# zhangyp15/MonoFlex

Hardware: AMD Instinct MI355X
Metric: images/sec at 1280x384, DLA-34+DCNv2 forward+decode (higher is better)
Workload: dtype bf16; 1 GPU; DLA-34+DCNv2+9 heads+edge fusion forward + NMS/top-K/3D decode, batch 8 per GPU, 1280x384, bf16 (BASELINE.json configs[1]); batch_per_gpu=8, launch=hipGraph, parallelism=replicas x1 (no collective on the inference path), sub_batch_streams=1, detections_last_step=400, h2d_excluded=True, d2h_excluded=True

## Files before the change

### include/monoflex_hip.h

```cpp
#ifndef MONOFLEX_HIP_H
#define MONOFLEX_HIP_H

#include <stddef.h>
#include <stdint.h>

#ifdef __cplusplus
extern "C" {
#endif

#define MFX_ABI_VERSION 3

enum { MFX_F32 = 0, MFX_BF16 = 1, MFX_F16 = 2 ,
       MFX_F16X2 = 3  };
enum { MFX_ACT_NONE = 0, MFX_ACT_RELU = 1, MFX_ACT_LEAKY = 2 , MFX_ACT_DCN_OFFMASK = 3  };
enum { MFX_OK = 0, MFX_ERR_ARG = -1, MFX_ERR_UNSUPPORTED = -2, MFX_ERR_LAUNCH = -3, MFX_ERR_WORKSPACE = -4 };

int mfx_abi_version(void);
const char* mfx_last_error(void);
int mfx_set_option(const char* name, int value);
int mfx_reset_options(void);
int mfx_commit_options(void);
long mfx_get_counter(const char* name);

int mfx_f16x2_range_check(int reset);
// ... 111 lines not shown
int mfx_nchw_to_nhwc(const float* x, void* y, int B, int C, int H, int W, int ldy, int dtype, void* stream);
int mfx_nhwc_to_nchw(const void* x, float* y, int B, int C, int H, int W, int ldx, int dtype, void* stream);
int mfx_pack_image_nhwc4(const float* x, void* y, int B, int H, int W, int pad_h, int pad_w_left, int pad_w_right,
                         int dtype, void* stream);

typedef struct {
    const void* x;
    const void* w1;
    const float* scale1; const float* shift1;
    const void* w2;
    const float* bias2;
    float* out;
    float* planar;
    int32_t B, H, W, nbranch, K_pad, ld_out, dtype, planar_c;
    int32_t ch_off[16]; int32_t c_out[16];
    float w2_scale[16];
    const void* w1_32; const void* w2_32;
} mfx_heads_desc;
int mfx_heads_fused(const mfx_heads_desc* d, void* stream);

int mfx_edge_scatter_add(float* out, int ld_out, int ch_off, int C, const float* v, int ldv,
                         const int32_t* edge_xy, const int32_t* edge_len, int B, int L, int H, int W,
                         float* planar , void* stream);

size_t mfx_decode_topk_workspace_bytes(int ncls, int B, int K);
int mfx_decode_topk(const float* hmap, long b_stride, long c_stride, long p_stride, int ncls, int B, int H, int W, int K,
                    float* scores, int32_t* index, void* workspace, size_t workspace_bytes, void* stream);

int mfx_decode_boxes(const float* hmap, int ld, int reg_off, const float* scores, const int32_t* index,
                     int ncls, int B, int H, int W, int K, const float* calib, const int32_t* pad,
                     const int32_t* img_size, float threshold, float* det, float* topk, int32_t* valid,
                     void* stream);
enum { MFX_DEPTH_SOFT = 0, MFX_DEPTH_HARD = 1, MFX_DEPTH_MEAN = 2, MFX_DEPTH_DIRECT = 3, MFX_DEPTH_KEYPOINTS_AVG = 4,
       MFX_DEPTH_KEYPOINTS_CENTER = 5, MFX_DEPTH_KEYPOINTS_02 = 6, MFX_DEPTH_KEYPOINTS_13 = 7 };
int mfx_decode_boxes_mode(const float* hmap, int ld, int reg_off, const float* scores, const int32_t* index,
                          int ncls, int B, int H, int W, int K, const float* calib, const int32_t* pad,
                          const int32_t* img_size, float threshold, int depth_mode, float* det, float* topk, int32_t* valid,
                          void* stream);
typedef struct mfx_decode_cfg {
    float dim_mean[9], dim_std[9];
    float depth_ref[2], depth_range[2];
    float down_ratio, eps;
    int depth_decode;
    int dim_exp, dim_use_std;
    int uncertainty_as_conf;
    int output_depth;
// ... 235 lines not shown
```

### monoflex_amd/build.py

```python
import hashlib
import os
import subprocess
import sys
from concurrent.futures import ThreadPoolExecutor

HERE = os.path.dirname(os.path.abspath(__file__))
CSRC = os.path.join(HERE, "csrc")
OBJ = os.path.join(CSRC, "build")
LIB = os.path.join(CSRC, "libmonoflex_hip.so")
SOURCES = ["capi.hip", "options.hip", "conv_kernels.hip", "conv_halo.hip", "conv_cw.hip", "conv_cws.hip", "misc_kernels.hip", "stem.hip", "f1_fused.hip", "heads.hip", "decode.hip", "dcn_wave.hip", "dcn_patch.hip", "dcn_lds.hip", "dcn_ps.hip", "gemm_as.hip", "dcn_ext.hip", "dcn_bwd.hip", "dcn_bwd_tile.hip", "psroi_pool.hip", "train_kernels.hip", "adamw.hip", "wgrad_tr.hip", "loss_kernels.hip", "box3d_iou.hip", "head_sparse.hip", "gram_heads.hip", "kitti_encode.hip", "kitti_eval.hip"]
FLAGS = ["--offload-arch=gfx950", "-O3", "-std=c++17", "-fPIC", "-Wall", "-Wno-unused-function"]
if os.environ.get("MFX_PROBES") == "1":
    FLAGS.append("-DMFX_PROBES")
EXTRA_FLAGS = {"kitti_encode.hip": ["-ffp-contract=off"], "kitti_eval.hip": ["-ffp-contract=off"],
               "dcn_bwd_tile.hip": ["-fno-slp-vectorize"]}


def _hipcc():
    return "/opt/rocm/bin/hipcc" if os.path.exists("/opt/rocm/bin/hipcc") else "hipcc"


def _headers_digest():
    h = hashlib.sha1()
    for root in (CSRC, os.path.join(os.path.dirname(HERE), "include")):
        for fn in sorted(os.listdir(root)):
            if fn.endswith(".h"):
                with open(os.path.join(root, fn), "rb") as f:
                    h.update(fn.encode() + f.read())
    return h.hexdigest()


def _source_stamp(src, headers):
    h = hashlib.sha1()
# ... 47 lines not shown
```

### monoflex_amd/csrc/options.h

```cpp
#pragma once

#define MFX_NOLO (-2147483647 - 1)
#define MFX_NOHI 2147483647

#define MFX_OPTION_LIST(X) \
     \
    X(conv_tile, 0, MFX_NOLO, MFX_NOHI, "implicit-GEMM tile of mfx_conv2d_nhwc: 0 = automatic, else a tile id (conv_kernels.hip: 1 = 256x16, 2 = 256x32, 3 = 128x64, " \
        "4 = 64x64, 5 = 128x128, 6 = 64x128, 7 = 256x64, 8 = 256x128 / 8 waves, 9 = 128x128 / 8 waves), taken where it fits Cout_pad") \
    X(dcn_tile, 0, MFX_NOLO, MFX_NOHI, "the same for the fused gather DCN kernel") \
    X(cat_tile, 0, MFX_NOLO, MFX_NOHI, "the same for mfx_cat_conv1x1_nhwc") \
    X(kc, 0, MFX_NOLO, MFX_NOHI, "16-byte chunks per LDS row of the implicit-GEMM main loop: 0 = automatic (8 where K_pad allows), 4 = force 4") \
    X(ksplit, 0, MFX_NOLO, MFX_NOHI, "split-K of mfx_conv2d_nhwc: 0 = automatic (never: measured neutral-to-slower on DLA level4/5), 1 = never split, " \
        "n = force n splits where legal") \
    X(dcn_ksplit, 0, MFX_NOLO, MFX_NOHI, "the same for the fused DCN kernel") \
    X(halo, 1, MFX_NOLO, MFX_NOHI, "LDS-staged halo kernels for 3x3 convs: 0 = generic kernel only, 1 = automatic, >= 2 = force variant (value - 1)") \
    X(halo_cg, 0, MFX_NOLO, MFX_NOHI, "max channels per patch pass of the halo kernel (0 = default)") \
    X(halo_s2, 1, MFX_NOLO, MFX_NOHI, "0 = stride-2 3x3 convs stay on the generic implicit-GEMM kernel") \
    X(halo_pair, 1, MFX_NOLO, MFX_NOHI, "split precision walks K in step pairs where mfx_conv_desc.w_frag_pair is given (0 = two mma_chunk per pair)") \
    X(halo_cw, 1, MFX_NOLO, MFX_NOHI, "0 = conv3x3_wave_kernel only, 1 = the compile-time-geometry kernel (conv_cw.hip) where an instantiation exists") \
    X(cw_rows6, 1, MFX_NOLO, MFX_NOHI, "0 = 8-row tiles everywhere in conv_cw.hip (1: 6-row tiles where Ho % 6 == 0, Ho % 8 != 0, Ho <= 48)") \
    X(halo_cws, 1, MFX_NOLO, MFX_NOHI, "0 = conv3x3_wave_kernel<f32s_t> only, 1 = the compile-time-geometry split-precision kernel (conv_cws.hip) where an instantiation exists") \
     \
    X(dcn_wave, 1, MFX_NOLO, MFX_NOHI, "0 = first-generation kernel only, 1 = automatic, 2.. = force variant") \
    X(dcn_patch, 1, MFX_NOLO, MFX_NOHI, "LDS-patch DCN kernel: 0 = off, 1 = automatic, 2 = force (FM 4), 3 = force FM 2, 4 = force FM 1, 5-7 = wide margin FM 4/2/1, " \
        "8 = padded layout") \
    X(dcn_patch_fn8, 1, MFX_NOLO, MFX_NOHI, "1 = one workgroup of the LDS-patch kernel covers 128 output channels where Cout_pad % 128 == 0") \
    X(dcn_fuse_off, 1, MFX_NOLO, MFX_NOHI, "1 = the LDS-patch kernel computes the offset/mask conv itself where the caller supplies its weights") \
    X(dcn_lds, 1, MFX_NOLO, MFX_NOHI, "0 = off, 1 = automatic (64 -> 64 on large 16-bit maps), 2 = wherever the kernel applies") \
    X(dcn_lds_rows, 16, MFX_NOLO, MFX_NOHI, "tile rows, 16 | 8 (three workgroups per CU; measured slower: 2.570 vs 2.551 ms per step, profiles/r06_dcn_lds.md)") \
     \
    X(heads_persist, 1, MFX_NOLO, MFX_NOHI, "1 = one workgroup per resident slot (n > 1: n workgroups), each a contiguous range of (tile, branch) units; " \
        "0 = one workgroup per tile.  B=8 bf16: 516 -> 503 us (tools/probes/heads_probe.py), bit-identical output") \
    X(heads_mfma32, 0, MFX_NOLO, MFX_NOHI, "1 = the v_mfma_f32_32x32x16 form of the kernel where the caller supplies its packs (mfx_heads_desc.w1_32 / w2_32)") \
    X(heads_planes, 0, MFX_NOLO, MFX_NOHI, "1 = four k-group planes (no LDS bank conflicts: 48 % -> 11 % of the LDS cycles, LDS-active cycles -42 %), " \
        "0 = one 144-byte record per pixel.  Same kernel time (555 vs 555 us, A/B in one run): not LDS-bound") \
    X(topk_strips, 8, MFX_NOLO, MFX_NOHI, "row strips per (class, image) map when a workspace is supplied; 1 = single-workgroup kernel") \
    X(topk_merge_z, 16, MFX_NOLO, MFX_NOHI, "workgroups per (class, image) map in the merge; values outside 1..64 are an error") \
    X(topk_merge_threads, 512, MFX_NOLO, MFX_NOHI, "their size; must be a multiple of 64 in 64..512 (the merge ranks by whole wavefronts; 512 = its __launch_bounds__)") \
     \
    X(wgrad_mfma, 1, MFX_NOLO, MFX_NOHI, "0 = VALU kernel for bf16 too, 1 = 64x64 MFMA tiles, 3 = 128x128 where they fit") \
    X(wgrad_blocks, 600, MFX_NOLO, MFX_NOHI, "target workgroup count of the MFMA weight-gradient kernel (measured, B=8 step: 64 -> 146 ms, 150 -> 90, 300 -> 78, " \
        "600 -> 73, 2048 -> 75, 8192 -> 81: the tile atomics of every slab cost more than the extra workgroups hide)") \
    X(wgrad_ws, 1, MFX_NOLO, MFX_NOHI, "0 = always accumulate the tiles with atomics") \
    X(wgrad_ws_blocks, 1200, MFX_NOLO, MFX_NOHI, "target workgroup count when partial tiles go to the workspace (step: 1200 -> 58.0 ms, 2400 -> 58.3, 4800 -> 58.6; " \
        "atomics: 59.6)") \
    X(wgrad_min_m, 128, MFX_NOLO, MFX_NOHI, "fewest pixels of a slab of the MFMA weight-gradient kernel.  r06: 1024 left the 1x1 / Root layers of the 24x80 and 12x40 " \
        "maps with 8-16 slabs (120-240 workgroups of 32 iterations each: 31 us per layer for 4 GFLOP); same-box step 17.50 (1024) / 17.31 (512) / 17.27 (256) / " \
        "17.23-17.31 (128) / 17.26 (64) ms") \
    X(wgrad_tr, 1, MFX_NOLO, MFX_NOHI, "0 = first-generation kernel everywhere (2: the transposed-read kernel also where Cout % 128 != 0)") \
    X(wgrad_tr_blocks, 512, 1, MFX_NOHI, "target workgroup count (tiles x pixel slabs)") \
    X(wgrad_patch, 1, MFX_NOLO, MFX_NOHI, "0 = off (the 3x3 / s1 / p1 weight-gradient form with the input patch in LDS)") \
    X(wgrad_patch_blocks, 256, 1, MFX_NOHI, "target workgroup count") \
    X(wgrad_patch_waves, 12, MFX_NOLO, MFX_NOHI, "6 (64 x 96 block per wave) or 12 (64 x 48)") \
    X(stem_wgrad_blocks, 512, 1, MFX_NOHI, "target workgroup count of the stem's weight-gradient kernel (mfx_stem_wgrad_16)") \
     \
    X(bn_apply_blocks, 1024, MFX_NOLO, MFX_NOHI, "workgroup cap of the two-launch forms' streaming kernels") \
    X(bn_blocks, 768, MFX_NOLO, MFX_NOHI, "target workgroup count of the column reductions (BN statistics / backward sums / bias sums)") \
    X(bn_onepass, 3, MFX_NOLO, MFX_NOHI, "bit 0 = backward, bit 1 = forward in one launch where the map fits (0 = the two-launch forms everywhere)") \
// ... 14 lines not shown
     \
    X(deterministic, 0, MFX_NOLO, MFX_NOHI, "any non-zero value = 1: every floating-point reduction of the training path runs in a fixed order (single-writer partial " \
        "sums, one pixel slab per weight-gradient tile, 64-bit fixed-point accumulation of the DCN input gradient) so that two runs -- eager or replayed from a " \
        "hipGraph -- produce bit-identical results.  Slower; the default (0) keeps the atomics")

#define MFX_PROBE_OPTION_LIST(X) \
    X(dcn_bt_dbg, 0, MFX_NOLO, MFX_NOHI, "experiment switches of dcn_bwd_tile_kernel (0 in production)") \
    X(heads_dbg, 0, MFX_NOLO, MFX_NOHI, "timing probes of the bf16 heads kernel (see DBG in heads.hip)")

#define MFX_COUNTER_LIST(X) \
     \
    X(dcn_lds, "launches of the fourth-generation DCN kernel (dcn_lds.hip) on 16-bit maps") \
    X(dcn_lds_of, "those of dcn_lds that computed the offset/mask conv themselves") \
    X(dcn_lds_split, "launches of dcn_lds.hip in split precision (not counted in dcn_lds)") \
    X(dcn_patch, "launches of the third-generation, LDS-patch DCN kernel (dcn_patch.hip)") \
    X(dcn_wave, "launches of the second-generation DCN kernel (dcn_wave.hip)") \
    X(dcn_gather, "launches of the first-generation fused gather DCN kernel (conv_kernels.hip)") \
    X(conv_cw, "launches of the compile-time-geometry 3x3 kernel (conv_cw.hip)") \
    X(conv_cws, "launches of its split-precision form (conv_cws.hip)") \
    X(conv_halo, "launches of the LDS-staged halo kernel (conv_halo.hip)") \
    X(conv_igemm, "launches of the generic implicit-GEMM kernel (conv_kernels.hip)") \
    X(conv_splitk, "those that ran split-K") \
    X(conv_bn_stats, "convolutions whose epilogue accumulated the BatchNorm statistics") \
     \
    X(wgrad_patch, "weight gradients by the LDS-patch kernel (wgrad_tr.hip)") \
    X(wgrad_tr, "weight gradients by the transposed-read kernel (wgrad_tr.hip)") \
    X(wgrad_mfma, "weight gradients by the first-generation MFMA kernel (train_kernels.hip)") \
    X(wgrad_valu, "weight gradients by the VALU kernel") \
    X(wgrad_reduce, "launches of the pass that sums their partial tiles (wgrad_reduce_kernel)") \
    X(stem_wgrad, "launches of the stem's weight-gradient kernel") \
    X(bn_fwd_onepass, "train-mode BatchNorm forwards in one launch") \
    X(bn_bwd_onepass, "BatchNorm backwards in one launch") \
    X(bn_fwd_two, "BatchNorm forwards in the two-launch form") \
    X(bn_bwd_two, "BatchNorm backwards in the two-launch form") \
    X(dcn_bt_fly, "DCN backward calls that took the gcol-free form") \
    X(dcn_bt_fused, "launches of dcn_bwd_sample_wgrad_kernel") \
    X(dcn_bt_tile, "launches of dcn_bwd_tile_kernel") \
    X(dcn_bt_sample, "launches of dcn_bwd_sample_kernel") \
    X(dcn_bt_far, "launches of dcn_bwd_far_kernel + dcn_bwd_far_fly_kernel") \
    X(gram, "phase calls of mfx_gram_heads on 16-bit maps") \
    X(adamw_multi, "calls of mfx_adamw_multi")

#define MFX_DECLARE_OPTION(name, def, lo, hi, doc) extern int g_opt_##name;
#define MFX_DECLARE_COUNTER(name, doc) extern long g_cnt_##name;
MFX_OPTION_LIST(MFX_DECLARE_OPTION)
MFX_PROBE_OPTION_LIST(MFX_DECLARE_OPTION)
// ... 4 lines not shown
```

### monoflex_amd/lib.py

```python
import ctypes
import os

HERE = os.path.dirname(os.path.abspath(__file__))
LIB_PATH = os.environ.get("MFX_LIB_PATH") or os.path.join(HERE, "csrc", "libmonoflex_hip.so")

MFX_F32, MFX_BF16, MFX_F16, MFX_F16X2 = 0, 1, 2, 3
ACT_NONE, ACT_RELU, ACT_LEAKY, ACT_DCN_OFFMASK = 0, 1, 2, 3
MAX_SEG = 9

c_int, c_void_p, c_float, c_size_t = ctypes.c_int32, ctypes.c_void_p, ctypes.c_float, ctypes.c_size_t


class ConvDesc(ctypes.Structure):
    _fields_ = [("x", c_void_p), ("w", c_void_p), ("w_frag", c_void_p), ("scale", c_void_p), ("shift", c_void_p), ("res", c_void_p),
                ("y", c_void_p), ("rowmap", c_void_p),
                ("B", c_int), ("H", c_int), ("W", c_int), ("x_pixstride", c_int), ("Ck", c_int),
                ("kh", c_int), ("kw", c_int), ("stride", c_int), ("pad_h", c_int), ("pad_w", c_int), ("dil_w", c_int),
                ("Ho", c_int), ("Wo", c_int), ("M", c_int), ("Cout", c_int), ("Cout_pad", c_int), ("K_pad", c_int),
                ("ldy", c_int), ("ldres", c_int), ("act", c_int), ("dtype", c_int), ("out_dtype", c_int),
                ("workspace", c_void_p), ("workspace_bytes", ctypes.c_int64),
                ("stats", c_void_p), ("stats_ncopy", c_int), ("stats_done", ctypes.POINTER(c_int)), ("w_frag_pair", c_void_p)]


class CatDesc(ctypes.Structure):
# ... 2 lines not shown
                ("w", c_void_p), ("scale", c_void_p), ("shift", c_void_p), ("res", c_void_p), ("y", c_void_p),
                ("M", c_int), ("Cout", c_int), ("Cout_pad", c_int), ("K_pad", c_int), ("ldy", c_int),
                ("ldres", c_int), ("act", c_int), ("dtype", c_int)]


class DcnDesc(ctypes.Structure):
    _fields_ = [("x", c_void_p), ("offmask", c_void_p), ("w", c_void_p), ("scale", c_void_p), ("shift", c_void_p),
                ("y", c_void_p), ("w_frag", c_void_p),
                ("B", c_int), ("H", c_int), ("W", c_int), ("C", c_int),
                ("kh", c_int), ("kw", c_int), ("stride", c_int), ("pad", c_int), ("dil", c_int),
                ("Ho", c_int), ("Wo", c_int), ("Cout", c_int), ("Cout_pad", c_int), ("K_pad", c_int),
                ("ldy", c_int), ("act", c_int), ("dtype", c_int), ("w_frag_f16", c_void_p),
                ("workspace", c_void_p), ("workspace_bytes", ctypes.c_int64),
                ("off_w_frag_f16", c_void_p), ("off_shift", c_void_p), ("offmask_out", c_void_p),
                ("nonsquare", c_int), ("stride_w", c_int), ("pad_w", c_int), ("dil_w", c_int), ("w_pair_f16", c_void_p)]


class HeadsDesc(ctypes.Structure):
    _fields_ = [("x", c_void_p), ("w1", c_void_p), ("scale1", c_void_p), ("shift1", c_void_p), ("w2", c_void_p),
                ("bias2", c_void_p), ("out", c_void_p), ("planar", c_void_p),
                ("B", c_int), ("H", c_int), ("W", c_int), ("nbranch", c_int), ("K_pad", c_int), ("ld_out", c_int),
                ("dtype", c_int), ("planar_c", c_int), ("ch_off", c_int * 16), ("c_out", c_int * 16), ("w2_scale", ctypes.c_float * 16),
                ("w1_32", c_void_p), ("w2_32", c_void_p)]


class KittiDesc(ctypes.Structure):
    _fields_ = [(n, c_void_p) for n in (
        "records", "n_obj", "P", "img_wh", "flip", "hm", "cls_ids", "target_centers", "keypoints", "keypoints_depth_mask",
        "dimensions", "locations", "reg_mask", "reg_weight", "offset_3D", "bboxes", "gt_bboxes", "rotys", "trunc_mask", "alphas",
        "orientations", "occlusions", "truncations", "pad_size", "edge_indices", "edge_len", "P_out", "heat_radius", "status")] + \
        [(n, c_int) for n in ("B", "max_objs", "in_w", "in_h", "down", "num_classes")] + \
        [(n, ctypes.c_double) for n in ("filter_trunc", "filter_size", "edge_ratio")]


class KittiEvalDesc(ctypes.Structure):
    _fields_ = [(n, c_void_p) for n in ("gt", "dt", "gt_off", "dt_off", "pair_off", "classes", "min_overlaps", "overlaps", "tp_scores",
                                        "num_valid_gt", "thresholds", "num_thresholds", "pr")] + \
        [(n, c_int) for n in ("B", "n_gt", "n_dt", "num_classes", "num_k", "compute_aos")] + [("n_pairs", ctypes.c_int64)]


class AdamWDesc(ctypes.Structure):
    _fields_ = [("p", c_void_p), ("g", c_void_p), ("m", c_void_p), ("v", c_void_p), ("step", c_void_p), ("numel", ctypes.c_longlong),
                ("group", c_int), ("pad_", c_int)]


class AdamWGroup(ctypes.Structure):
# ... 53 lines not shown
    "mfx_reset_options": (_I, []),
    "mfx_commit_options": (_I, []),
    "mfx_get_counter": (ctypes.c_long, [ctypes.c_char_p]),
    "mfx_f16x2_range_check": (ctypes.c_int, [ctypes.c_int]),
    "mfx_dcn_v2_workspace_bytes": (_S, [_I] * 14),
    "mfx_dcn_v2_workspace_bytes_g": (_S, [_I] * 15),
    "mfx_dcn_v2_forward": (_I, [_P] * 6 + [_I] * 14 + [_P, _S, _P]),
    "mfx_dcn_v2_backward": (_I, [_P] * 11 + [_I] * 14 + [_P, _S, _P]),
    "mfx_dcn_v2_psroi_pooling_forward": (_I, [_P] * 5 + [_I] * 8 + [_F] + [_I] * 5 + [_F, _P]),
    "mfx_dcn_v2_psroi_pooling_backward": (_I, [_P] * 7 + [_I] * 8 + [_F] + [_I] * 5 + [_F, _P]),
    "mfx_conv2d_nhwc": (_I, [ctypes.POINTER(ConvDesc), _P]),
    "mfx_cat_conv1x1_nhwc": (_I, [ctypes.POINTER(CatDesc), _P]),
    "mfx_dcn_nhwc": (_I, [ctypes.POINTER(DcnDesc), _P]),
    "mfx_dcn_sample_nhwc": (_I, [_P, _P, _P, _P, _P, _I, _I, _I, _I, _I, _I, _I, _P]),
    "mfx_project_nhwc": (_I, [_P, _P, _P, _I, _I, _I, _I, _I, _I, _P]),
    "mfx_maxpool2x2_nhwc": (_I, [_P, _P, _I, _I, _I, _I, _I, _P]),
    "mfx_upsample_add_nhwc": (_I, [_P, _P, _P, _P, _I, _I, _I, _I, _I, _I, _P]),
    "mfx_nchw_to_nhwc": (_I, [_P, _P, _I, _I, _I, _I, _I, _I, _P]),
    "mfx_nhwc_to_nchw": (_I, [_P, _P, _I, _I, _I, _I, _I, _I, _P]),
    "mfx_pack_image_nhwc4": (_I, [_P, _P, _I, _I, _I, _I, _I, _I, _I, _P]),
    "mfx_heads_fused": (_I, [ctypes.POINTER(HeadsDesc), _P]),
    "mfx_dcn_fuses_offset_conv": (_I, [ctypes.POINTER(DcnDesc)]),
    "mfx_edge_scatter_add": (_I, [_P, _I, _I, _I, _P, _I, _P, _P, _I, _I, _I, _I, _P, _P]),
    "mfx_decode_topk_workspace_bytes": (_S, [_I, _I, _I]),
    "mfx_decode_topk": (_I, [_P, ctypes.c_long, ctypes.c_long, ctypes.c_long, _I, _I, _I, _I, _I, _P, _P, _P, _S, _P]),
    "mfx_conv_wgrad_nhwc": (_I, [_P, _P, _P] + [_I] * 15 + [_P]),
    "mfx_conv_wgrad_nhwc_dil": (_I, [_P, _P, _P] + [_I] * 16 + [_P]),
    "mfx_conv_wgrad_oihw": (_I, [_P, _P, _P] + [_I] * 17 + [_P, _S, _P]),
    "mfx_pack_conv_weight": (_I, [_P, _I, _I, _I, _I, _I, _P, _P, _I, _I, _I, _I, _P]),
    "mfx_adamw_chunk_elems": (_I, []),
    "mfx_adamw_multi": (_I, [_P, _P, _I, ctypes.c_longlong, _P, _P, _P]),
    "mfx_colsum": (_I, [_P, _P, ctypes.c_long, _I, _I, _I, _P]),
    "mfx_colsum_add": (_I, [_P, _P, ctypes.c_long, _I, _I, _I, _P]),
    "mfx_bn_stats": (_I, [_P, _P, _P, ctypes.c_long, _I, _I, _P]),
    "mfx_bn_finalize": (_I, [_P, _P, _P, _P, _P, _P, _F, _F, ctypes.c_long, _P, _P, _P, _P, _I, _P]),
    "mfx_bn_act_fwd": (_I, [_P, _P, _P, _P, _P, ctypes.c_long, _I, _I, _I, _P]),
    "mfx_bn_act_bwd": (_I, [_P] * 10 + [ctypes.c_long, _I, _I, _I, _P]),
    "mfx_stem_wgrad_bf16": (_I, [_P, _P, _P, _I, _I, _I, _I, _I, _P, _S, _P]),
    "mfx_stem_wgrad_16": (_I, [_P, _P, _P, _I, _I, _I, _I, _I, _I, _P, _S, _P]),
    "mfx_pack_chunk_elems": (_I, []),
    "mfx_pack_conv_weights_batched": (_I, [_P, _P, _I, ctypes.c_longlong, _I, _P]),
    "mfx_head_sparse_fwd": (_I, [ctypes.POINTER(HeadSparseDesc), _P]),
    "mfx_head_sparse_bwd": (_I, [ctypes.POINTER(HeadSparseDesc), _P]),
    "mfx_gram_heads": (_I, [ctypes.POINTER(GramDesc), _I, _P]),
    "mfx_bn_train_stats": (_I, [_P] * 6 + [_F, _F, ctypes.c_long, _I, _I, _P, _P, _P, _I, _P]),
    "mfx_bn_scratch_bytes": (_S, []),
# ... 130 lines not shown
```

### monoflex_amd/model/head/detector_predictor.py

```python
import numpy as np
import torch
from torch import nn

from ... import autograd as AG
from ... import lib as L
from ... import ops

HM_LD = 64
REG_OFF = 8


GRAM_HEADS = [__import__("os").environ.get("MFX_GRAM_HEADS", "1") != "0"]
GRAM_OFFSET = [__import__("os").environ.get("MFX_GRAM_OFFSET", "1") != "0"]


class InPlaceABN(nn.Module):

    def __init__(self, num_features, eps=1e-5, momentum=0.1, affine=True, activation="leaky_relu", activation_param=0.01):
        super().__init__()
        if not affine:
            raise NotImplementedError("InPlaceABN holder: affine=True only")
        self.num_features, self.eps, self.momentum, self.affine, self.track_running_stats = num_features, eps, momentum, True, True
        self.weight = nn.Parameter(torch.ones(num_features))
        self.bias = nn.Parameter(torch.zeros(num_features))
# ... 78 lines not shown
        lasts = [[self.class_head[2]]] + [list(h) for h in self.reg_heads]
        c_out = [sum(h.weight.shape[0] for h in heads) for heads in lasts]
        ch_off = [0] + [REG_OFF + sum(c_out[1:i]) for i in range(1, len(lasts))]
        assert ch_off[-1] + c_out[-1] <= HM_LD
        p = ops.pack_heads([t[0].weight for t in trunks], [self._abn_fold(t[1]) for t in trunks],
                           [torch.cat([h.weight for h in heads]) for heads in lasts], [torch.cat([h.bias for h in heads]) for heads in lasts],
                           self.num_classes, ch_off, HM_LD, dtype)
        if self.enable_edge_fusion:
            oi = self.offset_index[0]
            w_e = torch.cat((self.class_head[0].weight, self.reg_features[oi][0].weight), 0)
            s0, b0 = self._abn_fold(self.class_head[1])
            s1, b1 = self._abn_fold(self.reg_features[oi][1])
            p.edge_trunk = ops.pack_conv(w_e, dtype, torch.cat((s0, s1)), torch.cat((b0, b1)), stride=1, pad=1, act=L.ACT_LEAKY)
            p.edge_branches = []
            for seq, cout, choff in ((self.trunc_heatmap_conv, self.num_classes, 0),
                                     (self.trunc_offset_conv, 2, REG_OFF + sum(sum(c) for c in self.regression_channel_cfg[:oi])
                                      + sum(self.regression_channel_cfg[oi][:self.offset_index[1]]))):
                c1, bn, c3 = seq[0], seq[1], seq[3]
                scale, shift = ops.fold_bn(bn, c1.bias)
                pk1 = ops.pack_conv(c1.weight.detach().unsqueeze(2), dtype, scale, shift, stride=1, pad=0,
                                    act=L.ACT_RELU if self.edge_fusion_relu else L.ACT_NONE)
                pk2 = ops.pack_conv(c3.weight.detach().unsqueeze(2), dtype, None, c3.bias, stride=1, pad=0, act=L.ACT_NONE, cout=4)
                p.edge_branches.append((pk1, pk2, cout, choff))
        self._packs[key] = p
        return p

    def forward_nhwc(self, features, edge_indices=None, edge_lens=None, edge_rowmap=None):
        if self.training:
            raise RuntimeError("forward_nhwc is the fused eval path; training goes through forward_train")
        p = self._pack(ops.compute_tag(self, features.dtype))
        hm, planar = ops.heads_fused(features, p, planar_classes=self.num_classes)
        self.last_cls_planar = planar
        if self.enable_edge_fusion:
            if edge_indices is None:
                raise ValueError("edge fusion is enabled: targets must carry edge_indices / edge_len")
            B, H, W, _ = features.shape
            Lmax = edge_indices.shape[1]
            rowmap = edge_rowmap if edge_rowmap is not None else make_edge_rowmap(edge_indices, H, W)
            trunk = ops.conv2d(features, p.edge_trunk, rowmap=rowmap)
            trunk = trunk.view(B, 1, Lmax + 2, 2 * self.head_conv)
            for bi, (pk1, pk2, cout, choff) in enumerate(p.edge_branches):
                f1 = ops.conv2d(trunk, pk1, x_ch_off=bi * self.head_conv)
                o = ops.conv2d(f1, pk2, out_dtype=torch.float32)
                ops.edge_scatter_add(hm, choff, cout, o, edge_indices, edge_lens, planar=planar if choff == 0 else None)
        return hm

    def forward_train(self, features, edge_indices=None, edge_lens=None, object_rows=None, plan=None):
        B, H, W, _ = features.shape
        trunks = [self.class_head] + list(self.reg_features)
        lasts = [[self.class_head[2]]] + [list(h) for h in self.reg_heads]
        oi = self.offset_index[0]
        sparse = object_rows is not None
        feats, outs, sp = [], [], []
        gram = sparse and GRAM_HEADS[0]
        fuse_nodes = self.enable_edge_fusion and self.fused_edge_nodes
        gram_off = gram and GRAM_OFFSET[0] and (fuse_nodes or not self.enable_edge_fusion)
        is_sparse = lambda bi: sparse and bi != 0 and (bi - 1 != oi or gram_off)
        dense_ids = [bi for bi in range(len(trunks)) if not (gram and is_sparse(bi))]
        ys = dict(zip(dense_ids, AG.fanout_conv(features, [trunks[bi][0].weight for bi in dense_ids], 1)))
        edge_rows = {}
# ... 180 lines not shown
```

### monoflex_amd/ops.py

```python
import ctypes
import os
from typing import Optional

import torch

from . import lib as L
from .packing import (F16X2, STEM_PAD_H, STEM_PAD_WL, STEM_PAD_WR, PackedCat, PackedConv, PackedHeads, _elems, _pad_rows_cols, _pow2,
                      _round_up, add_f16_fragments, cast_operand, compute_tag, cout_pad, dcn_pair_fragments, dcn_ps_pack, fold_bn, fragment_major,
                      pack_cat, pack_conv, pack_heads, pack_stem, pack_upsample, pair_steps, split_chunks, split_halves, split_weight_scale, storage_dtype)


def _stream():
    return ctypes.c_void_p(torch.cuda.current_stream().cuda_stream)


def _first_cuda_device(args):
    for a in args:
        if torch.is_tensor(a):
            if a.is_cuda:
                return a.device
        elif isinstance(a, (list, tuple)):
            d = _first_cuda_device(a)
            if d is not None:
                return d
    return None


def on_tensor_device(fn):
    import functools

    @functools.wraps(fn)
    def run(*args, **kwargs):
# ... 271 lines not shown
@on_tensor_device
def heads_fused(x, p: PackedHeads, planar_classes=0):
    _need_cuda(x)
    B, H, W, C = x.shape
    assert C == 64
    out = torch.empty((B, H, W, p.ld_out), dtype=torch.float32, device=x.device)
    planar = torch.empty((B, planar_classes, H * W), dtype=torch.float32, device=x.device) if planar_classes else None
    d = L.HeadsDesc()
    d.planar, d.planar_c = (planar.data_ptr() if planar is not None else None), planar_classes
    d.x, d.w1, d.scale1, d.shift1 = x.data_ptr(), p.w1.data_ptr(), p.scale1.data_ptr(), p.shift1.data_ptr()
    d.w2, d.bias2, d.out = p.w2.data_ptr(), p.bias2.data_ptr(), out.data_ptr()
    d.w1_32 = p.w1_32.data_ptr() if p.w1_32 is not None else None
    d.w2_32 = p.w2_32.data_ptr() if p.w2_32 is not None else None
    d.B, d.H, d.W, d.nbranch, d.K_pad, d.ld_out = B, H, W, len(p.c_out), p.K_pad, p.ld_out
    d.dtype = L.MFX_F16X2 if p.split else _dt(x.dtype)
    for i, (o, c) in enumerate(zip(p.ch_off, p.c_out)):
        d.ch_off[i], d.c_out[i] = o, c
        d.w2_scale[i] = p.w2_scale[i] if p.w2_scale is not None else 1.0
    L.check(L.load().mfx_heads_fused(ctypes.byref(d), _stream()), "mfx_heads_fused")
    return out, planar


@on_tensor_device
def edge_scatter_add(out, ch_off, C, v, edge_xy, edge_len, planar=None):
    _need_cuda(out, v, edge_xy, edge_len, planar)
    B, H, W, ld = out.shape
    Lmax = edge_xy.shape[1]
    L.check(L.load().mfx_edge_scatter_add(_ptr(out), ld, ch_off, C, _ptr(v), v.shape[-1], _ptr(edge_xy), _ptr(edge_len),
                                          B, Lmax, H, W, _ptr(planar), _stream()), "mfx_edge_scatter_add")


@on_tensor_device
def decode_topk(hmap, ch_off, ncls, K, planar=None):
    _need_cuda(hmap, planar)
    B, H, W, ld = hmap.shape
    scores = torch.empty((B, ncls, K), dtype=torch.float32, device=hmap.device)
    index = torch.empty((B, ncls, K), dtype=torch.int32, device=hmap.device)
    if planar is not None:
        src, bs, cs, ps = planar.data_ptr(), ncls * H * W, H * W, 1
    else:
        src, bs, cs, ps = hmap.data_ptr() + 4 * ch_off, H * W * ld, 1, ld
    lib = L.load()
    ws = torch.empty(int(lib.mfx_decode_topk_workspace_bytes(ncls, B, K)), dtype=torch.uint8, device=hmap.device)
    L.check(lib.mfx_decode_topk(ctypes.c_void_p(src), bs, cs, ps, ncls, B, H, W, K, _ptr(scores), _ptr(index), _ptr(ws), ws.numel(),
                                _stream()), "mfx_decode_topk")
    return scores, index
# ... 172 lines not shown
```

### monoflex_amd/packing.py

```python
import math
from dataclasses import dataclass
from typing import Optional

import torch

from .lib import ACT_NONE, ACT_RELU


F16X2 = "f16x2"


def compute_tag(module, dtype):
    if dtype == torch.float32 and module.__dict__.get("_mfx_split", False):
        return F16X2
    return dtype


def storage_dtype(dtype):
    return torch.float32 if dtype == F16X2 else dtype


def _elems(dtype):
    return 4 if (dtype == torch.float32 or dtype == F16X2) else 8

# ... 90 lines not shown
    Cout_pad: int
    K_pad: int
    act: int
    split: bool = False


@dataclass
class PackedHeads:
    w1: torch.Tensor
    scale1: torch.Tensor
    shift1: torch.Tensor
    w2: torch.Tensor
    bias2: torch.Tensor
    K_pad: int
    ch_off: list
    c_out: list
    ld_out: int
    split: bool = False
    w2_scale: Optional[list] = None
    w1_32: Optional[torch.Tensor] = None
    w2_32: Optional[torch.Tensor] = None
    edge_trunk: Optional[PackedConv] = None
    edge_branches: Optional[list] = None


def fragment_major(w2d, dtype):
    E = _elems(dtype)
    N, K = w2d.shape
    assert N % 16 == 0 and K % (4 * E) == 0
    return w2d.view(N // 16, 16, K // (4 * E), 4, E).permute(0, 2, 3, 1, 4).contiguous()


def fold_bn(bn, conv_bias=None):
    scale = bn.weight.detach().float() / torch.sqrt(bn.running_var.detach().float() + bn.eps)
    shift = bn.bias.detach().float() - bn.running_mean.detach().float() * scale
    if conv_bias is not None:
        shift = shift + conv_bias.detach().float() * scale
    return scale.contiguous(), shift.contiguous()


def _pad_rows_cols(w2d, rows, cols):
    out = w2d.new_zeros(rows, cols)
    out[:w2d.shape[0], :w2d.shape[1]] = w2d
    return out


def pack_conv(weight, dtype, scale=None, shift=None, stride=1, pad=0, act=ACT_NONE, cout=None):
    Cout, Cin, kh, kw = weight.shape
    if not _pow2(Cin) or Cin < _elems(dtype):
        raise ValueError("pack_conv: Cin must be a power of two >= %d (got %d)" % (_elems(dtype), Cin))
    cout = Cout if cout is None else cout
    K_pad, cp, frag = operand_geometry(kh, kw, Cin, cout, stride, pad, pad, _elems(dtype))
    w2 = weight.detach().float().permute(0, 2, 3, 1).reshape(Cout, kh * kw * Cin)
# ... 147 lines not shown
```

Baseline: 3262 images/s.

## Fuse edge-fusion conv chain (trunk, Conv1d, 1x1) into one kernel

Adds a single HIP kernel that runs the edge fusion's 3x3 trunk conv over gathered edge pixels, then the k=3 Conv1d and the 1x1 output conv for both branches. Intermediates stay in LDS, and a register ring prefetches weights. It replaces five separate implicit-GEMM launches and their global-memory round trips of intermediate activations, and is enabled by default for the 16-bit configuration. The cost is a large LDS footprint per workgroup and a specialized shape, with a fallback to the old path otherwise.

```diff
diff --git a/include/monoflex_hip.h b/include/monoflex_hip.h
--- a/include/monoflex_hip.h
+++ b/include/monoflex_hip.h
@@ -157,6 +157,21 @@
 int mfx_edge_scatter_add(float* out, int ld_out, int ch_off, int C, const float* v, int ldv,
                          const int32_t* edge_xy, const int32_t* edge_len, int B, int L, int H, int W,
                          float* planar , void* stream);
+
+typedef struct {
+    const void* x;
+    const int32_t* edge_xy;
+    const void* w_trunk;
+    const float* scale_trunk; const float* shift_trunk;
+    const void* w_conv;
+    const float* scale_conv; const float* shift_conv;
+    const void* w_out;
+    const float* bias_out;
+    float* out;
+    int32_t B, H, W, C, L, head_conv, ksize, relu , dtype;
+} mfx_edge_chain_desc;
+int mfx_edge_chain(const mfx_edge_chain_desc* d, void* stream);
+int mfx_edge_chain_applies(const mfx_edge_chain_desc* d);
 
 size_t mfx_decode_topk_workspace_bytes(int ncls, int B, int K);
 int mfx_decode_topk(const float* hmap, long b_stride, long c_stride, long p_stride, int ncls, int B, int H, int W, int K,
diff --git a/monoflex_amd/build.py b/monoflex_amd/build.py
--- a/monoflex_amd/build.py
+++ b/monoflex_amd/build.py
@@ -8,7 +8,7 @@
 CSRC = os.path.join(HERE, "csrc")
 OBJ = os.path.join(CSRC, "build")
 LIB = os.path.join(CSRC, "libmonoflex_hip.so")
-SOURCES = ["capi.hip", "options.hip", "conv_kernels.hip", "conv_halo.hip", "conv_cw.hip", "conv_cws.hip", "misc_kernels.hip", "stem.hip", "f1_fused.hip", "heads.hip", "decode.hip", "dcn_wave.hip", "dcn_patch.hip", "dcn_lds.hip", "dcn_ps.hip", "gemm_as.hip", "dcn_ext.hip", "dcn_bwd.hip", "dcn_bwd_tile.hip", "psroi_pool.hip", "train_kernels.hip", "adamw.hip", "wgrad_tr.hip", "loss_kernels.hip", "box3d_iou.hip", "head_sparse.hip", "gram_heads.hip", "kitti_encode.hip", "kitti_eval.hip"]
+SOURCES = ["capi.hip", "options.hip", "conv_kernels.hip", "conv_halo.hip", "conv_cw.hip", "conv_cws.hip", "misc_kernels.hip", "stem.hip", "f1_fused.hip", "heads.hip", "edge_chain.hip", "decode.hip", "dcn_wave.hip", "dcn_patch.hip", "dcn_lds.hip", "dcn_ps.hip", "gemm_as.hip", "dcn_ext.hip", "dcn_bwd.hip", "dcn_bwd_tile.hip", "psroi_pool.hip", "train_kernels.hip", "adamw.hip", "wgrad_tr.hip", "loss_kernels.hip", "box3d_iou.hip", "head_sparse.hip", "gram_heads.hip", "kitti_encode.hip", "kitti_eval.hip"]
 FLAGS = ["--offload-arch=gfx950", "-O3", "-std=c++17", "-fPIC", "-Wall", "-Wno-unused-function"]
 if os.environ.get("MFX_PROBES") == "1":
     FLAGS.append("-DMFX_PROBES")
diff --git a/monoflex_amd/csrc/edge_chain.hip b/monoflex_amd/csrc/edge_chain.hip
--- /dev/null
+++ b/monoflex_amd/csrc/edge_chain.hip
@@ -0,0 +1,200 @@
+#include "../../include/monoflex_hip.h"
+#include "err.h"
+#include "common.h"
+
+namespace mfx {
+
+namespace ec {
+constexpr int SEG = 62, ROWS = 64;
+constexpr int CIN = 64, HC = 256;
+constexpr int NK1 = 9 * CIN / 32, NK2 = 3 * HC / 32, NK3 = HC / 32;
+constexpr int G_ROW = 9 * CIN * 2 + 16;
+constexpr int T_ROW = HC * 2 + 16;
+constexpr int G_BYTES = ROWS * G_ROW;
+constexpr int T_BYTES = (ROWS + 2) * T_ROW;
+constexpr int XY_BYTES = ROWS * 8;
+constexpr int SMEM = G_BYTES + T_BYTES + XY_BYTES;
+constexpr int DEPTH = 6;
+static_assert(ROWS * T_ROW <= G_BYTES, "the Conv1d output reuses the gathered input's space");
+}
+
+struct EdgeChainArgs {
+    const void* x; const int* edge_xy;
+    const void* w_trunk; const float* scale_trunk; const float* shift_trunk;
+    const void* w_conv; const float* scale_conv; const float* shift_conv;
+    const void* w_out; const float* bias_out;
+    float* out;
+    int B, H, W, L, relu;
+};
+
+template <int NK> __device__ __forceinline__ void ring_load(u32x4 (&slot)[4], const u32x4* wl, int ks) {
+#pragma unroll
+    for (int j = 0; j < 4; ++j) slot[j] = wl[(j * NK + ks) * 64];
+}
+
+template <int NK> __device__ __forceinline__ void ring_fill(u32x4 (&ring)[ec::DEPTH][4], const u32x4* wl) {
+#pragma unroll
+    for (int s = 0; s < ec::DEPTH; ++s)
+        if (s < NK) ring_load<NK>(ring[s], wl, s);
+}
+
+template <typename T, int NK, int ROWB, typename AF>
+__device__ __forceinline__ void chain_gemm(f32x4 (&acc)[4][4], u32x4 (&ring)[ec::DEPTH][4], const u32x4* wl, AF a_addr) {
+#pragma unroll
+    for (int i = 0; i < 4; ++i)
+#pragma unroll
+        for (int j = 0; j < 4; ++j) acc[i][j] = f32x4{0.f, 0.f, 0.f, 0.f};
+#pragma unroll
+    for (int ks = 0; ks < NK; ++ks) {
+        u32x4 a[4], b[4];
+#pragma unroll
+        for (int j = 0; j < 4; ++j) b[j] = ring[ks % ec::DEPTH][j];
+        if (ks + ec::DEPTH < NK) ring_load<NK>(ring[ks % ec::DEPTH], wl, ks + ec::DEPTH);
+        const char* ap = a_addr(ks);
+#pragma unroll
+        for (int i = 0; i < 4; ++i) a[i] = *reinterpret_cast<const u32x4*>(ap + i * 16 * ROWB);
+#pragma unroll
+        for (int i = 0; i < 4; ++i)
+#pragma unroll
+            for (int j = 0; j < 4; ++j) mma_chunk<T>(a[i], b[j], acc[i][j]);
+    }
+}
+
+template <typename T, int ACT>
+__device__ __forceinline__ void chain_epilogue(const f32x4 (&acc)[4][4], char* dst, const float* scale, const float* shift, int n0, int lane) {
+#pragma unroll
+    for (int j = 0; j < 4; ++j) {
+        const int n = n0 + j * 16 + (lane & 15);
+        const float sc = scale[n], sh = shift[n];
+#pragma unroll
+        for (int i = 0; i < 4; ++i) {
+            const int m = i * 16 + (lane >> 4) * 4;
+#pragma unroll
+            for (int r = 0; r < 4; ++r) {
+                float v = acc[i][j][r] * sc + sh;
+                if (ACT == ACT_RELU) v = fmaxf(v, 0.f);
+                if (ACT == ACT_LEAKY) v = v > 0.f ? v : 0.01f * v;
+                asm volatile("" : "+v"(v));
+                ElemTraits<T>::store(reinterpret_cast<T*>(dst + (m + r) * ec::T_ROW) + n, v);
+            }
+        }
+    }
+}
+
+template <typename T>
+__global__ __launch_bounds__(256) void edge_chain_kernel(EdgeChainArgs a) {
+    using namespace ec;
+    extern __shared__ __attribute__((aligned(16))) char smem[];
+    char* Gs = smem;
+    char* Ts = smem + G_BYTES;
+    int* xy = reinterpret_cast<int*>(smem + G_BYTES + T_BYTES);
+    const int tid = threadIdx.x, lane = tid & 63, wave = tid >> 6;
+    const int seg = blockIdx.x, br = blockIdx.y, b = blockIdx.z;
+    const int p0 = seg * SEG;
+
+    u32x4 ring[DEPTH][4];
+    const u32x4* w1 = reinterpret_cast<const u32x4*>(a.w_trunk) + (size_t)(br * 16 + wave * 4) * NK1 * 64 + lane;
+    ring_fill<NK1>(ring, w1);
+
+    if (tid < ROWS) {
+        const int p = min(max(p0 - 1 + tid, 0), a.L - 1);
+        const int* e = a.edge_xy + ((size_t)b * a.L + p) * 2;
+        xy[2 * tid] = min(max(e[0], 0), a.W - 1);
+        xy[2 * tid + 1] = min(max(e[1], 0), a.H - 1);
+    }
+    __syncthreads();
+    {
+        const char* xb = reinterpret_cast<const char*>(a.x) + (size_t)b * a.H * a.W * (CIN * 2);
+        constexpr int PER = ROWS * 72 / 256;
+        u32x4 g[PER];
+#pragma unroll
+        for (int i = 0; i < PER; ++i) {
+            const int idx = tid + 256 * i, row = idx / 72, rem = idx - row * 72, tap = rem >> 3, c = rem & 7;
+            const int th = tap / 3, tw = tap - th * 3;
+            const int ih = xy[2 * row + 1] + th - 1, iw = xy[2 * row] + tw - 1;
+            const bool ok = ih >= 0 && ih < a.H && iw >= 0 && iw < a.W;
+            const int ihc = min(max(ih, 0), a.H - 1), iwc = min(max(iw, 0), a.W - 1);
+            const u32x4 z = *reinterpret_cast<const u32x4*>(xb + ((size_t)ihc * a.W + iwc) * (CIN * 2) + c * 16);
+            g[i] = ok ? z : u32x4{0u, 0u, 0u, 0u};
+        }
+#pragma unroll
+        for (int i = 0; i < PER; ++i) {
+            const int idx = tid + 256 * i, row = idx / 72, rem = idx - row * 72;
+            *reinterpret_cast<u32x4*>(Gs + row * G_ROW + rem * 16) = g[i];
+        }
+    }
+    __syncthreads();
+
+    const int frag = (lane & 15), kq16 = (lane >> 4) * 16;
+    f32x4 acc[4][4];
+    chain_gemm<T, NK1, G_ROW>(acc, ring, w1, [&](int ks) { return Gs + frag * G_ROW + ks * 64 + kq16; });
+    const u32x4* w2 = reinterpret_cast<const u32x4*>(a.w_conv) + (size_t)(br * 16 + wave * 4) * NK2 * 64 + lane;
+    ring_fill<NK2>(ring, w2);
+    chain_epilogue<T, ACT_LEAKY>(acc, Ts, a.scale_trunk + br * HC, a.shift_trunk + br * HC, wave * 64, lane);
+    __syncthreads();
+
+    chain_gemm<T, NK2, T_ROW>(acc, ring, w2, [&](int ks) { return Ts + (frag + (ks >> 3)) * T_ROW + (ks & 7) * 64 + kq16; });
+    if (a.relu) chain_epilogue<T, ACT_RELU>(acc, Gs, a.scale_conv + br * HC, a.shift_conv + br * HC, wave * 64, lane);
+    else chain_epilogue<T, ACT_NONE>(acc, Gs, a.scale_conv + br * HC, a.shift_conv + br * HC, wave * 64, lane);
+    __syncthreads();
+
+    const u32x4* w3 = reinterpret_cast<const u32x4*>(a.w_out) + (size_t)br * NK3 * 64 + lane;
+    u32x4 b3[NK3];
+#pragma unroll
+    for (int ks = 0; ks < NK3; ++ks) b3[ks] = w3[ks * 64];
+    f32x4 o = f32x4{0.f, 0.f, 0.f, 0.f};
+#pragma unroll
+    for (int ks = 0; ks < NK3; ++ks)
+        mma_chunk<T>(*reinterpret_cast<const u32x4*>(Gs + (wave * 16 + frag) * T_ROW + ks * 64 + kq16), b3[ks], o);
+    const int n = lane & 15;
+    if (n < 4) {
+        const float bias = a.bias_out[br * 16 + n];
+#pragma unroll
+        for (int r = 0; r < 4; ++r) {
+            const int i = wave * 16 + (lane >> 4) * 4 + r, p = p0 + i;
+            if (i < SEG && p < a.L) a.out[(((size_t)br * a.B + b) * a.L + p) * 4 + n] = o[r] + bias;
+        }
+    }
+}
+
+static bool edge_chain_supported(const mfx_edge_chain_desc* d) {
+    return (d->dtype == MFX_BF16 || d->dtype == MFX_F16) && d->C == ec::CIN && d->head_conv == ec::HC && d->ksize == 3;
+}
+
+template <typename T> static int launch_edge_chain(const EdgeChainArgs& a, hipStream_t st) {
+    auto k = edge_chain_kernel<T>;
+    static bool attr_set = false;
+    if (!attr_set) {
+        MFX_HIP_CHECK(hipFuncSetAttribute(reinterpret_cast<const void*>(k), hipFuncAttributeMaxDynamicSharedMemorySize, ec::SMEM));
+        attr_set = true;
+    }
+    const int nseg = (a.L + ec::SEG - 1) / ec::SEG;
+    hipLaunchKernelGGL(k, dim3(nseg, 2, a.B), dim3(256), ec::SMEM, st, a);
+    MFX_HIP_CHECK(hipGetLastError());
+    return MFX_OK;
+}
+
+}
+using namespace mfx;
+
+extern "C" int mfx_edge_chain_applies(const mfx_edge_chain_desc* d) { return (d && g_opt_edge_chain != 0 && edge_chain_supported(d)) ? 1 : 0; }
+
+extern "C" int mfx_edge_chain(const mfx_edge_chain_desc* d, void* stream) {
+    if (!d || !d->x || !d->edge_xy || !d->w_trunk || !d->scale_trunk || !d->shift_trunk || !d->w_conv || !d->scale_conv || !d->shift_conv ||
+        !d->w_out || !d->bias_out || !d->out)
+        return mfx_fail(MFX_ERR_ARG, "edge_chain: null pointer");
+    if (d->dtype != MFX_BF16 && d->dtype != MFX_F16) return mfx_fail(MFX_ERR_UNSUPPORTED, "edge_chain: bf16 or fp16 activations only");
+    if (!edge_chain_supported(d)) return mfx_fail(MFX_ERR_UNSUPPORTED, "edge_chain: built for 64 feature channels, 256 head channels and a k = 3 Conv1d");
+    if (d->B <= 0 || d->H <= 0 || d->W <= 0 || d->L < 0) return mfx_fail(MFX_ERR_ARG, "edge_chain: bad B / H / W / L");
+    if (d->B > 65535) return mfx_fail(MFX_ERR_UNSUPPORTED, "edge_chain: more than 65535 images");
+    if (d->L == 0) return MFX_OK;
+    EdgeChainArgs a;
+    a.x = d->x; a.edge_xy = d->edge_xy;
+    a.w_trunk = d->w_trunk; a.scale_trunk = d->scale_trunk; a.shift_trunk = d->shift_trunk;
+    a.w_conv = d->w_conv; a.scale_conv = d->scale_conv; a.shift_conv = d->shift_conv;
+    a.w_out = d->w_out; a.bias_out = d->bias_out; a.out = d->out;
+    a.B = d->B; a.H = d->H; a.W = d->W; a.L = d->L; a.relu = d->relu ? 1 : 0;
+    ++g_cnt_edge_chain;
+    hipStream_t st = reinterpret_cast<hipStream_t>(stream);
+    return d->dtype == MFX_BF16 ? launch_edge_chain<bf16_t>(a, st) : launch_edge_chain<half_t>(a, st);
+}
diff --git a/monoflex_amd/csrc/options.h b/monoflex_amd/csrc/options.h
--- a/monoflex_amd/csrc/options.h
+++ b/monoflex_amd/csrc/options.h
@@ -34,6 +34,8 @@
     X(heads_mfma32, 0, MFX_NOLO, MFX_NOHI, "1 = the v_mfma_f32_32x32x16 form of the kernel where the caller supplies its packs (mfx_heads_desc.w1_32 / w2_32)") \
     X(heads_planes, 0, MFX_NOLO, MFX_NOHI, "1 = four k-group planes (no LDS bank conflicts: 48 % -> 11 % of the LDS cycles, LDS-active cycles -42 %), " \
         "0 = one 144-byte record per pixel.  Same kernel time (555 vs 555 us, A/B in one run): not LDS-bound") \
+    X(edge_chain, 1, MFX_NOLO, MFX_NOHI, "1 = the edge fusion's conv chain (trunk, Conv1d, 1x1 of both branches) as one kernel where mfx_edge_chain applies " \
+        "(edge_chain.hip: 16-bit modes, bit-identical output), 0 = five mfx_conv2d_nhwc launches") \
     X(topk_strips, 8, MFX_NOLO, MFX_NOHI, "row strips per (class, image) map when a workspace is supplied; 1 = single-workgroup kernel") \
     X(topk_merge_z, 16, MFX_NOLO, MFX_NOHI, "workgroups per (class, image) map in the merge; values outside 1..64 are an error") \
     X(topk_merge_threads, 512, MFX_NOLO, MFX_NOHI, "their size; must be a multiple of 64 in 64..512 (the merge ranks by whole wavefronts; 512 = its __launch_bounds__)") \
@@ -94,6 +96,7 @@
     X(conv_igemm, "launches of the generic implicit-GEMM kernel (conv_kernels.hip)") \
     X(conv_splitk, "those that ran split-K") \
     X(conv_bn_stats, "convolutions whose epilogue accumulated the BatchNorm statistics") \
+    X(edge_chain, "launches of the edge fusion's one-kernel conv chain (edge_chain.hip)") \
      \
     X(wgrad_patch, "weight gradients by the LDS-patch kernel (wgrad_tr.hip)") \
     X(wgrad_tr, "weight gradients by the transposed-read kernel (wgrad_tr.hip)") \
diff --git a/monoflex_amd/lib.py b/monoflex_amd/lib.py
--- a/monoflex_amd/lib.py
+++ b/monoflex_amd/lib.py
@@ -48,6 +48,12 @@
                 ("B", c_int), ("H", c_int), ("W", c_int), ("nbranch", c_int), ("K_pad", c_int), ("ld_out", c_int),
                 ("dtype", c_int), ("planar_c", c_int), ("ch_off", c_int * 16), ("c_out", c_int * 16), ("w2_scale", ctypes.c_float * 16),
                 ("w1_32", c_void_p), ("w2_32", c_void_p)]
+
+
+class EdgeChainDesc(ctypes.Structure):
+    _fields_ = [(n, c_void_p) for n in ("x", "edge_xy", "w_trunk", "scale_trunk", "shift_trunk", "w_conv", "scale_conv", "shift_conv",
+                                        "w_out", "bias_out", "out")] + \
+        [(n, c_int) for n in ("B", "H", "W", "C", "L", "head_conv", "ksize", "relu", "dtype")]
 
 
 class KittiDesc(ctypes.Structure):
@@ -147,6 +153,8 @@
     "mfx_heads_fused": (_I, [ctypes.POINTER(HeadsDesc), _P]),
     "mfx_dcn_fuses_offset_conv": (_I, [ctypes.POINTER(DcnDesc)]),
     "mfx_edge_scatter_add": (_I, [_P, _I, _I, _I, _P, _I, _P, _P, _I, _I, _I, _I, _P, _P]),
+    "mfx_edge_chain": (_I, [ctypes.POINTER(EdgeChainDesc), _P]),
+    "mfx_edge_chain_applies": (_I, [ctypes.POINTER(EdgeChainDesc)]),
     "mfx_decode_topk_workspace_bytes": (_S, [_I, _I, _I]),
     "mfx_decode_topk": (_I, [_P, ctypes.c_long, ctypes.c_long, ctypes.c_long, _I, _I, _I, _I, _I, _P, _P, _P, _S, _P]),
     "mfx_conv_wgrad_nhwc": (_I, [_P, _P, _P] + [_I] * 15 + [_P]),
diff --git a/monoflex_amd/model/head/detector_predictor.py b/monoflex_amd/model/head/detector_predictor.py
--- a/monoflex_amd/model/head/detector_predictor.py
+++ b/monoflex_amd/model/head/detector_predictor.py
@@ -124,6 +124,7 @@
                                     act=L.ACT_RELU if self.edge_fusion_relu else L.ACT_NONE)
                 pk2 = ops.pack_conv(c3.weight.detach().unsqueeze(2), dtype, None, c3.bias, stride=1, pad=0, act=L.ACT_NONE, cout=4)
                 p.edge_branches.append((pk1, pk2, cout, choff))
+            p.edge_chain = ops.pack_edge_chain(p.edge_trunk, p.edge_branches)
         self._packs[key] = p
         return p
 
@@ -138,6 +139,11 @@
                 raise ValueError("edge fusion is enabled: targets must carry edge_indices / edge_len")
             B, H, W, _ = features.shape
             Lmax = edge_indices.shape[1]
+            chain = ops.edge_chain(features, edge_indices, p.edge_chain) if p.edge_chain is not None else None
+            if chain is not None:
+                for bi, (_, _, cout, choff) in enumerate(p.edge_branches):
+                    ops.edge_scatter_add(hm, choff, cout, chain[bi], edge_indices, edge_lens, planar=planar if choff == 0 else None)
+                return hm
             rowmap = edge_rowmap if edge_rowmap is not None else make_edge_rowmap(edge_indices, H, W)
             trunk = ops.conv2d(features, p.edge_trunk, rowmap=rowmap)
             trunk = trunk.view(B, 1, Lmax + 2, 2 * self.head_conv)
diff --git a/monoflex_amd/ops.py b/monoflex_amd/ops.py
--- a/monoflex_amd/ops.py
+++ b/monoflex_amd/ops.py
@@ -5,9 +5,10 @@
 import torch
 
 from . import lib as L
-from .packing import (F16X2, STEM_PAD_H, STEM_PAD_WL, STEM_PAD_WR, PackedCat, PackedConv, PackedHeads, _elems, _pad_rows_cols, _pow2,
+from .packing import (F16X2, STEM_PAD_H, STEM_PAD_WL, STEM_PAD_WR, PackedCat, PackedConv, PackedEdgeChain, PackedHeads, _elems, _pad_rows_cols, _pow2,
                       _round_up, add_f16_fragments, cast_operand, compute_tag, cout_pad, dcn_pair_fragments, dcn_ps_pack, fold_bn, fragment_major,
-                      pack_cat, pack_conv, pack_heads, pack_stem, pack_upsample, pair_steps, split_chunks, split_halves, split_weight_scale, storage_dtype)
+                      pack_cat, pack_conv, pack_edge_chain, pack_heads, pack_stem, pack_upsample, pair_steps, split_chunks, split_halves, split_weight_scale,
+                      storage_dtype)
 
 
 def _stream():
@@ -325,6 +326,28 @@
 
 
 @on_tensor_device
+def edge_chain(x, edge_xy, p: PackedEdgeChain):
+    _need_cuda(x, edge_xy)
+    B, H, W, C = x.shape
+    Lmax = edge_xy.shape[1]
+    if edge_xy.dtype != torch.int32 or not edge_xy.is_contiguous() or not x.is_contiguous() or x.dtype != p.w_trunk.dtype:
+        return None
+    d = L.EdgeChainDesc()
+    d.x, d.edge_xy = x.data_ptr(), edge_xy.data_ptr()
+    d.w_trunk, d.scale_trunk, d.shift_trunk = p.w_trunk.data_ptr(), p.scale_trunk.data_ptr(), p.shift_trunk.data_ptr()
+    d.w_conv, d.scale_conv, d.shift_conv = p.w_conv.data_ptr(), p.scale_conv.data_ptr(), p.shift_conv.data_ptr()
+    d.w_out, d.bias_out = p.w_out.data_ptr(), p.bias_out.data_ptr()
+    d.B, d.H, d.W, d.C, d.L, d.head_conv, d.ksize, d.relu, d.dtype = B, H, W, C, Lmax, 256, 3, int(p.relu), _dt(x.dtype)
+    lib = L.load()
+    if not lib.mfx_edge_chain_applies(ctypes.byref(d)):
+        return None
+    out = torch.empty((2, B, Lmax, 4), dtype=torch.float32, device=x.device)
+    d.out = out.data_ptr()
+    L.check(lib.mfx_edge_chain(ctypes.byref(d), _stream()), "mfx_edge_chain")
+    return out
+
+
+@on_tensor_device
 def edge_scatter_add(out, ch_off, C, v, edge_xy, edge_len, planar=None):
     _need_cuda(out, v, edge_xy, edge_len, planar)
     B, H, W, ld = out.shape
diff --git a/monoflex_amd/packing.py b/monoflex_amd/packing.py
--- a/monoflex_amd/packing.py
+++ b/monoflex_amd/packing.py
@@ -136,6 +136,20 @@
     w2_32: Optional[torch.Tensor] = None
     edge_trunk: Optional[PackedConv] = None
     edge_branches: Optional[list] = None
+    edge_chain: Optional["PackedEdgeChain"] = None
+
+
+@dataclass
+class PackedEdgeChain:
+    w_trunk: torch.Tensor
+    scale_trunk: torch.Tensor
+    shift_trunk: torch.Tensor
+    w_conv: torch.Tensor
+    scale_conv: torch.Tensor
+    shift_conv: torch.Tensor
+    w_out: torch.Tensor
+    bias_out: torch.Tensor
+    relu: bool
 
 
 def fragment_major(w2d, dtype):
@@ -143,6 +157,25 @@
     N, K = w2d.shape
     assert N % 16 == 0 and K % (4 * E) == 0
     return w2d.view(N // 16, 16, K // (4 * E), 4, E).permute(0, 2, 3, 1, 4).contiguous()
+
+
+def pack_edge_chain(trunk: PackedConv, branches):
+    dtype = trunk.w.dtype
+    if trunk.split or dtype not in (torch.bfloat16, torch.float16) or len(branches) != 2:
+        return None
+    if (trunk.kh, trunk.kw, trunk.Ck, trunk.Cout, trunk.K_pad) != (3, 3, 64, 512, 576):
+        return None
+    for pk1, pk2, cout, _ in branches:
+        if (pk1.kh, pk1.kw, pk1.Ck, pk1.Cout, pk1.K_pad) != (1, 3, 256, 256, 768) or pk1.act not in (ACT_NONE, ACT_RELU) or pk1.act != branches[0][0].act:
+            return None
+        if (pk2.kh, pk2.kw, pk2.Ck, pk2.Cout_pad, pk2.K_pad) != (1, 1, 256, 16, 256) or cout > 4 or pk2.scale is not None or pk2.act != ACT_NONE:
+            return None
+    return PackedEdgeChain(fragment_major(trunk.w, dtype), trunk.scale, trunk.shift,
+                           torch.stack([fragment_major(pk1.w, dtype) for pk1, _, _, _ in branches]).contiguous(),
+                           torch.stack([pk1.scale for pk1, _, _, _ in branches]).contiguous(),
+                           torch.stack([pk1.shift for pk1, _, _, _ in branches]).contiguous(),
+                           torch.stack([fragment_major(pk2.w, dtype) for _, pk2, _, _ in branches]).contiguous(),
+                           torch.stack([pk2.shift for _, pk2, _, _ in branches]).contiguous(), branches[0][0].act == ACT_RELU)
 
 
 def fold_bn(bn, conv_bias=None):
```

Result: faster. 3301 images/s, median of 6 (+1.2%).
